# JuliaPhysics/BeamletOptics.jl

Hardware: AMD Instinct MI355X
Metric: ray-surface intersections/s (higher is better)
Workload: dtype f64

## Files before the change

### beamletoptics.jl_amd/csrc/bmo_engine.hip

```cpp
#include <hip/hip_runtime.h>
#include <hipcub/hipcub.hpp>

#include <algorithm>
#include <cmath>
#include <chrono>
#include <cstdio>
#include <cstdlib>
#include <cstring>
#include <ctime>
#include <unistd.h>
#include <memory>
#include <mutex>
#include <string>
#include <map>
#include <vector>

#include "bmo_lane.hpp"

using namespace bmo;

namespace {

thread_local std::string g_err;
struct Knobs {
// ... 1274 lines not shown
        c0.d[L::OPL * cap + j] = 0.0;
    }
    c0.i[I_NODE * cap + j] = perm ? perm[j] : (int32_t)j;
    c0.i[I_K * cap + j] = 0;
    c0.i[I_HOBJ * cap + j] = -1;
    c0.i[I_HSHAPE * cap + j] = -1;
    c0.i[I_FLAGS * cap + j] = (1 < r_max) ? 0 : F_DEAD;
    if (KIND == BMO_BEAM_GAUSSIAN) {
        nodes.aux[j * 4 + 0] = cont ? planes[27 * n + j] : 0.0;
        nodes.aux[j * 4 + 1] = planes[20 * n + j];
        nodes.aux[j * 4 + 2] = planes[21 * n + j];
        nodes.aux[j * 4 + 3] = planes[22 * n + j];
    }
    nodes.root[j] = (int32_t)j;
    nodes.parent[j] = -1;
    nodes.nseg[j] = 1;
    nodes.status[j] = 0;
    nodes.li[j] = lambda_idx[j];
    nodes.lambda[j] = planes[(KIND == BMO_BEAM_GAUSSIAN ? 18 : 6) * n + j];
    nodes.hit_det[j] = -1;
    nodes.key[j] = 0;
    if (nodes.tbits) nodes.tbits[j] = 1ull;
}
__global__ void bin_planes_kernel(const double* __restrict__ in, const int32_t* __restrict__ perm, int64_t n, int n_planes, double* __restrict__ out) {
    const int64_t s = (int64_t)blockIdx.x * blockDim.x + threadIdx.x;
    if (s >= n) return;
    const int64_t j = perm[s];
    for (int p = 0; p < n_planes; ++p) out[(int64_t)p * n + s] = in[(int64_t)p * n + j];
}

__global__ void old_obj_scatter_kernel(Chunk c, int32_t chunk_index, const int32_t* __restrict__ rec_start, int32_t* __restrict__ rec_obj,
                                       int64_t* __restrict__ rec_loc) {
    const int64_t j = (int64_t)blockIdx.x * blockDim.x + threadIdx.x;
    if (j >= c.count) return;
    const int32_t node = chunk_node(c, j);
    if (node < 0) return;
    const int32_t k = c.i[I_K * c.cap + j];
    rec_obj[(int64_t)rec_start[node] + k] = c.i[I_OBJ * c.cap + j];
    rec_loc[(int64_t)rec_start[node] + k] = ((int64_t)chunk_index << OLD_LOC_SHIFT) | j;
}
__global__ void old_first_child_kernel(const int32_t* __restrict__ parent, const unsigned long long* __restrict__ key, int64_t n, int32_t* __restrict__ first_child) {
    const int64_t c = (int64_t)blockIdx.x * blockDim.x + threadIdx.x;
    if (c >= n) return;
    const int32_t p = parent[c];
    if (p >= 0 && !(key[c] & 1ull)) first_child[p] = (int32_t)c;
}
constexpr int MAX_PATH_LEVELS = 26;
__global__ void pack_keys_kernel(const int32_t* __restrict__ root_of, const unsigned long long* __restrict__ key, int64_t n, int bits_depth, int bits_path,
                                 uint32_t* __restrict__ k32, unsigned long long* __restrict__ k64) {
    const int64_t i = (int64_t)blockIdx.x * blockDim.x + threadIdx.x;
    if (i >= n) return;
    const unsigned long long k = key[i];
    const unsigned long long root = (unsigned long long)root_of[i], depth = k >> 32, path = k & ((1ull << bits_path) - 1ull);
    const unsigned long long packed = (root << (bits_depth + bits_path)) | (depth << bits_path) | path;
    if (k32) k32[i] = (uint32_t)packed;
    else k64[i] = packed;
}
constexpr int MAX_HEAP_LEVELS = 5;
__device__ __forceinline__ unsigned heap_index(unsigned long long key) {
    const unsigned depth = (unsigned)(key >> 32);
    return (1u << depth) - 1u + (unsigned)(key & ((1ull << depth) - 1ull));
}
__global__ void tree_bits_kernel(const int32_t* __restrict__ root_of, const unsigned long long* __restrict__ key, int64_t n, unsigned long long* __restrict__ bits) {
    const int64_t i = (int64_t)blockIdx.x * blockDim.x + threadIdx.x;
    if (i >= n) return;
    atomicOr(&bits[root_of[i]], 1ull << heap_index(key[i]));
}
__global__ void tree_count_kernel(const unsigned long long* __restrict__ bits, int64_t n_roots, int32_t* __restrict__ cnt) {
    const int64_t r = (int64_t)blockIdx.x * blockDim.x + threadIdx.x;
    if (r < n_roots) cnt[r] = __popcll(bits[r]);
}
__global__ void tree_rank_kernel(const int32_t* __restrict__ root_of, const unsigned long long* __restrict__ key, int64_t n, const unsigned long long* __restrict__ bits,
                                 const int32_t* __restrict__ base, int32_t* __restrict__ order) {
    const int64_t i = (int64_t)blockIdx.x * blockDim.x + threadIdx.x;
    if (i >= n) return;
    const int32_t r = root_of[i];
    const unsigned h = heap_index(key[i]);
    order[base[r] + __popcll(bits[r] & ((1ull << h) - 1ull))] = (int32_t)i;
}
__global__ void node_depth_kernel(const unsigned long long* __restrict__ key, int64_t n, uint32_t* __restrict__ depth) {
    const int64_t i = (int64_t)blockIdx.x * blockDim.x + threadIdx.x;
    if (i < n) depth[i] = (uint32_t)(key[i] >> 32);
}
__global__ void level_starts_kernel(const uint32_t* __restrict__ sorted_depth, int64_t n, int64_t max_depth, int32_t* __restrict__ start) {
    const int64_t i = (int64_t)blockIdx.x * blockDim.x + threadIdx.x;
    if (i >= n) return;
    const int64_t d = sorted_depth[i], dprev = i ? (int64_t)sorted_depth[i - 1] : -1;
    for (int64_t x = dprev + 1; x <= d; ++x) start[x] = (int32_t)i;
    if (i == n - 1)
        for (int64_t x = d + 1; x <= max_depth + 1; ++x) start[x] = (int32_t)n;
}
__global__ void level_root_rank_kernel(const int32_t* __restrict__ ids, int32_t cnt, int32_t* __restrict__ rank) {
    const int i = blockIdx.x * blockDim.x + threadIdx.x;
    if (i < cnt) rank[ids[i]] = i;
}
__global__ void level_flag_kernel(const int32_t* __restrict__ ids, int32_t cnt, const int32_t* __restrict__ parent, const unsigned long long* __restrict__ key,
                                  const int32_t* __restrict__ rank, int32_t* __restrict__ flag) {
    const int i = blockIdx.x * blockDim.x + threadIdx.x;
    if (i >= cnt) return;
    const int32_t nd = ids[i];
    if (!(key[nd] & 1ull)) flag[rank[parent[nd]]] = 1;
}
__global__ void level_rank_kernel(const int32_t* __restrict__ ids, int32_t cnt, const int32_t* __restrict__ parent, const unsigned long long* __restrict__ key,
                                  const int32_t* __restrict__ scan, int32_t* __restrict__ rank) {
    const int i = blockIdx.x * blockDim.x + threadIdx.x;
    if (i >= cnt) return;
    const int32_t nd = ids[i];
    rank[nd] = 2 * scan[rank[parent[nd]]] + (int32_t)(key[nd] & 1ull);
}
__global__ void gather_u32_kernel(const int32_t* __restrict__ idx, const int32_t* __restrict__ src, int64_t n, uint32_t* __restrict__ dst) {
    const int64_t i = (int64_t)blockIdx.x * blockDim.x + threadIdx.x;
    if (i < n) dst[i] = (uint32_t)src[idx[i]];
}
__global__ void root_depth_key_kernel(const int32_t* __restrict__ idx, const int32_t* __restrict__ root_of, const unsigned long long* __restrict__ key, int64_t n,
                                      int bits_depth, unsigned long long* __restrict__ out) {
    const int64_t i = (int64_t)blockIdx.x * blockDim.x + threadIdx.x;
    if (i >= n) return;
    const int32_t nd = idx[i];
    out[i] = ((unsigned long long)root_of[nd] << bits_depth) | (key[nd] >> 32);
}
__global__ void iota_kernel(int32_t* a, int64_t n) {
    const int64_t j = (int64_t)blockIdx.x * blockDim.x + threadIdx.x;
    if (j < n) a[j] = (int32_t)j;
}
__global__ void sweep_key_kernel(Chunk c, const int32_t* __restrict__ root, const int32_t* __restrict__ root_cfg, int64_t m, uint32_t* __restrict__ key,
                                 int32_t* __restrict__ slot) {
    const int64_t j = (int64_t)blockIdx.x * blockDim.x + threadIdx.x;
    if (j >= m) return;
    key[j] = (uint32_t)root_cfg[root[c.i[I_NODE * c.cap + j]]];
    slot[j] = (int32_t)j;
}
__global__ void sweep_bounds_kernel(const uint32_t* __restrict__ key, int64_t m, int32_t* __restrict__ beg, int32_t* __restrict__ end) {
    const int64_t i = (int64_t)blockIdx.x * blockDim.x + threadIdx.x;
    if (i >= m) return;
    const uint32_t k = key[i];
    if (i == 0 || key[i - 1] != k) beg[k] = (int32_t)i;
    if (i == m - 1 || key[i + 1] != k) end[k] = (int32_t)(i + 1);
}
__global__ void sweep_pad_kernel(const int32_t* __restrict__ beg, const int32_t* __restrict__ end, int32_t n_configs, int32_t* __restrict__ padded) {
    const int32_t c = (int32_t)(blockIdx.x * blockDim.x + threadIdx.x);
    if (c >= n_configs) return;
    padded[c] = (end[c] - beg[c] + 63) & ~63;
}
__global__ void sweep_scatter_kernel(const uint32_t* __restrict__ key, const int32_t* __restrict__ slot, int64_t m, const int32_t* __restrict__ beg,
                                     const int32_t* __restrict__ pstart, int64_t lanes, int32_t* __restrict__ map, unsigned long long* __restrict__ overflow) {
    const int64_t i = (int64_t)blockIdx.x * blockDim.x + threadIdx.x;
    if (i >= m) return;
    const uint32_t k = key[i];
    const int64_t v = (int64_t)pstart[k] + (i - beg[k]);
    if (v < lanes) map[v] = slot[i];
    else atomicAdd(overflow, 1ull);
}

__global__ void hit_flags_kernel(const int32_t* order, const int32_t* hit_det, int64_t n, int32_t n_det, int32_t nsub, int32_t* flags) {
    const int64_t i = (int64_t)blockIdx.x * blockDim.x + threadIdx.x;
    if (i >= n) return;
    const int32_t d = hit_det[order[i]];
    for (int32_t q = 0; q < n_det; ++q) flags[(int64_t)q * n + i] = (q == d) ? nsub : 0;
}
__global__ void hit_offsets_kernel(const int32_t* __restrict__ offs, const int32_t* __restrict__ flags, int64_t n, int32_t n_det, int32_t* __restrict__ out) {
    const int d = (int)threadIdx.x;
    if (d < n_det) out[d] = offs[(int64_t)d * n];
    if (d == n_det) out[d] = offs[(int64_t)n_det * n - 1] + flags[(int64_t)n_det * n - 1];
}
__global__ void hit_gather_kernel(const int32_t* __restrict__ order, const int32_t* __restrict__ hit_det, const double* __restrict__ hit, int64_t n, int32_t nsub,
                                  const int32_t* __restrict__ offs, int64_t cap, double* __restrict__ out, int32_t* __restrict__ out_node,
                                  unsigned long long* __restrict__ overflow) {
    __shared__ int32_t s_nd[256], s_pos[256];
    const int64_t i0 = (int64_t)blockIdx.x * 256;
    {
        const int64_t i = i0 + threadIdx.x;
        int32_t nd = -1, pos = -1;
        if (i < n) {
            nd = order[i];
            const int32_t d = hit_det[nd];
            if (d >= 0) {
                pos = offs[(int64_t)d * n + i];
                if ((int64_t)pos + nsub > cap) {
                    atomicAdd(overflow, 1ull);
                    pos = -1;
                } else {
                    for (int q = 0; q < nsub; ++q) out_node[pos + q] = (int32_t)i;
                }
            }
        }
        s_nd[threadIdx.x] = nd;
        s_pos[threadIdx.x] = pos;
    }
    __syncthreads();
    const int width = 9 * nsub;
    const int de = 256 / width, dk = 256 % width;
    int e = (int)threadIdx.x / width, k = (int)threadIdx.x % width;
    for (int t = threadIdx.x; t < 256 * width; t += 256) {
        const int32_t pos = s_pos[e];
        if (pos >= 0) out[(int64_t)pos * 9 + k] = hit[(int64_t)s_nd[e] * width + k];
        e += de;
        k += dk;
        if (k >= width) {
            k -= width;
            e += 1;
        }
    }
}

__global__ void rank_kernel(const int32_t* __restrict__ order, int64_t n, int32_t* __restrict__ rank) {
    const int64_t i = (int64_t)blockIdx.x * blockDim.x + threadIdx.x;
    if (i < n) rank[order[i]] = (int32_t)i;
}
__global__ void canon_nodes_kernel(const int32_t* __restrict__ order, const int32_t* __restrict__ rank, int64_t n, int gaussian, const int32_t* __restrict__ root,
                                   const int32_t* __restrict__ parent, const int32_t* __restrict__ nseg, const int32_t* __restrict__ status,
                                   const unsigned long long* __restrict__ key, const double* __restrict__ lambda, const double* __restrict__ aux,
                                   int32_t* __restrict__ o_root, int32_t* __restrict__ o_parent, int32_t* __restrict__ o_first_child, int32_t* __restrict__ o_nseg,
                                   int32_t* __restrict__ o_status, double* __restrict__ o_aux) {
    const int64_t i = (int64_t)blockIdx.x * blockDim.x + threadIdx.x;
    if (i >= n) return;
    const int32_t nd = order[i];
    const int32_t p = parent[nd];
    o_root[i] = root[nd];
    o_parent[i] = p < 0 ? -1 : rank[p];
    o_nseg[i] = nseg[nd];
    o_status[i] = status[nd];
    if (gaussian) {
        o_aux[4 * i + 0] = aux[4 * (int64_t)nd + 1];
        o_aux[4 * i + 1] = aux[4 * (int64_t)nd + 2];
        o_aux[4 * i + 2] = aux[4 * (int64_t)nd + 3];
        o_aux[4 * i + 3] = lambda[nd];
    } else {
        o_aux[4 * i + 0] = lambda[nd];
        o_aux[4 * i + 1] = o_aux[4 * i + 2] = o_aux[4 * i + 3] = 0.0;
    }
    if (p >= 0 && !(key[nd] & 1ull)) o_first_child[rank[p]] = (int32_t)i;
}
__global__ void dst_base_kernel(const int32_t* __restrict__ order, const int32_t* __restrict__ first_rec, int64_t n, int32_t* __restrict__ dst_base) {
    const int64_t i = (int64_t)blockIdx.x * blockDim.x + threadIdx.x;
    if (i < n) dst_base[order[i]] = first_rec[i];
}
__global__ void last_records_kernel(Chunk c, int planes, const int32_t* __restrict__ rank, const int32_t* __restrict__ nseg, int64_t nn, double* __restrict__ rec,
                                    int32_t* __restrict__ obj, int32_t* __restrict__ shape) {
    const int64_t j = (int64_t)blockIdx.x * blockDim.x + threadIdx.x;
    if (j >= c.count) return;
    const int32_t nd = chunk_node(c, j);
    if (nd < 0) return;
    if (c.i[I_K * c.cap + j] != nseg[nd] - 1) return;
    const int64_t dst = rank[nd];
    for (int p = 0; p < planes; ++p) rec[(int64_t)p * nn + dst] = c.d[(int64_t)p * c.cap + j];
    obj[dst] = c.i[I_OBJ * c.cap + j];
    shape[dst] = c.i[I_SHAPE * c.cap + j];
}
__global__ void hit_columns_kernel(const double* __restrict__ src, int64_t n, int n_cols, double* __restrict__ dst) {
    const int64_t t = (int64_t)blockIdx.x * blockDim.x + threadIdx.x;
    if (t >= n * n_cols) return;
    const int64_t i = t / n_cols;
    dst[t] = src[i * 9 + (t - i * n_cols)];
}

__global__ void order_records_kernel(Chunk c, int planes, const int32_t* __restrict__ dst_base, int64_t nr, double* __restrict__ rec,
                                     int32_t* __restrict__ obj, int32_t* __restrict__ shape) {
    const int64_t j = (int64_t)blockIdx.x * blockDim.x + threadIdx.x;
    if (j >= c.count) return;
    const int32_t nd = chunk_node(c, j);
    if (nd < 0) return;
    const int64_t dst = (int64_t)dst_base[nd] + c.i[I_K * c.cap + j];
    for (int p = 0; p < planes; ++p) rec[(int64_t)p * nr + dst] = c.d[(int64_t)p * c.cap + j];
    obj[dst] = c.i[I_OBJ * c.cap + j];
    shape[dst] = c.i[I_SHAPE * c.cap + j];
}

struct PoolBlock {
    void* p;
    size_t bytes;
    int device;
};
std::mutex g_pool_mu;
std::vector<PoolBlock> g_pool;
size_t g_pool_bytes = 0;

void* pool_take(size_t bytes, int device, size_t& got) {
    std::lock_guard<std::mutex> lk(g_pool_mu);
    int best = -1;
    for (int i = 0; i < (int)g_pool.size(); ++i) {
        const PoolBlock& b = g_pool[i];
        if (b.device != device || b.bytes < bytes || b.bytes > bytes + bytes / 4 + 4096) continue;
        if (best < 0 || b.bytes < g_pool[best].bytes) best = i;
    }
    if (best < 0) return nullptr;
    void* p = g_pool[best].p;
    got = g_pool[best].bytes;
    g_pool_bytes -= got;
    g_pool.erase(g_pool.begin() + best);
    return p;
}
void pool_give(void* p, size_t bytes, int device) {
    std::lock_guard<std::mutex> lk(g_pool_mu);
    g_pool.push_back({p, bytes, device});
    g_pool_bytes += bytes;
}
void pool_release_all() {
    std::lock_guard<std::mutex> lk(g_pool_mu);
    int cur = 0;
    (void)hipGetDevice(&cur);
    for (auto& b : g_pool) {
        (void)hipSetDevice(b.device);
        (void)hipFree(b.p);
    }
    (void)hipSetDevice(cur);
    g_pool.clear();
    g_pool_bytes = 0;
}

struct PoolHold;
thread_local PoolHold* g_hold = nullptr;
void host_pool_give(void* p, size_t bytes);
struct PoolHold {
    hipStream_t stream;
    std::vector<PoolBlock> dev;
    std::vector<std::pair<void*, size_t>> host;
    PoolHold* prev;
    explicit PoolHold(hipStream_t s) : stream(s), prev(g_hold) { g_hold = this; }
    ~PoolHold() {
        g_hold = prev;
        (void)hipStreamSynchronize(stream);
        for (auto& b : dev) pool_give(b.p, b.bytes, b.device);
        for (auto& h : host) host_pool_give(h.first, h.second);
    }
    PoolHold(const PoolHold&) = delete;
    PoolHold& operator=(const PoolHold&) = delete;
    struct Now {
        PoolHold* saved;
        Now() : saved(g_hold) { g_hold = nullptr; }
        ~Now() { g_hold = saved; }
    };
};

struct DevBuf {
    void* p = nullptr;
    size_t bytes = 0;
// ... 1179 lines not shown
```

### beamletoptics.jl_amd/csrc/bmo_trace_host.inc.hpp

```cpp

struct DevCtx {
    hipStream_t stream = nullptr;
    hipEvent_t ev[4] = {nullptr, nullptr, nullptr, nullptr};
    Counters* pinned = nullptr;
    std::vector<hipEvent_t> step_ev;
    std::mutex busy;
};
int device_ctx(int device, DevCtx*& out) {
    static std::mutex ctx_mu;
    static std::vector<std::pair<int, std::unique_ptr<DevCtx>>> ctxs;
    std::lock_guard<std::mutex> lk(ctx_mu);
    for (auto& c : ctxs)
        if (c.first == device) {
            out = c.second.get();
            return BMO_OK;
        }
    auto nc = std::make_unique<DevCtx>();
    HIP_TRY(hipStreamCreateWithFlags(&nc->stream, hipStreamNonBlocking));
    for (int q = 0; q < 4; ++q) HIP_TRY(hipEventCreate(&nc->ev[q]));
    HIP_TRY(hipHostMalloc(reinterpret_cast<void**>(&nc->pinned), sizeof(Counters), hipHostMallocDefault));
    out = nc.get();
    ctxs.emplace_back(device, std::move(nc));
    return BMO_OK;
}
// ... 343 lines not shown
    const double span = (double)(t1 - t0);
    const int NB = 40;
    std::vector<double> busy(NB, 0.0);
    for (size_t w = 0; w < nw; ++w) {
        const double a = (double)(t[2 * w] - t0) / span * NB, b2 = (double)(t[2 * w + 1] - t0) / span * NB;
        for (int q = (int)a; q < NB && q <= (int)b2; ++q) busy[q] += std::min(b2, (double)q + 1) - std::max(a, (double)q);
    }
    fprintf(stderr, "[bmo] timeline step %d: %zu waves, span %.3f ms; mean waves at work per 1/%d of the span:\n ", steps, nw, span / 1e5, NB);
    for (int q = 0; q < NB; ++q) fprintf(stderr, " %.0f", busy[q]);
    fprintf(stderr, "\n");
    {
        std::vector<size_t> idx(nw);
        for (size_t w = 0; w < nw; ++w) idx[w] = w;
        const size_t top = std::min<size_t>(nw, 12);
        std::partial_sort(idx.begin(), idx.begin() + (long)top, idx.end(), [&](size_t a, size_t b2) { return t[2 * a + 1] > t[2 * b2 + 1]; });
        fprintf(stderr, "[bmo] timeline step %d: last waves to end (wave of the grid: start .. end in ms):", steps);
        for (size_t q = 0; q < top; ++q) fprintf(stderr, "  %zu: %.3f .. %.3f", idx[q], (double)(t[2 * idx[q]] - t0) / 1e5, (double)(t[2 * idx[q] + 1] - t0) / 1e5);
        fprintf(stderr, "\n");
        std::vector<double> dur(nw);
        for (size_t w = 0; w < nw; ++w) dur[w] = (double)(t[2 * w + 1] - t[2 * w]) / 1e5;
        std::vector<double> srt = dur;
        std::sort(srt.begin(), srt.end());
        fprintf(stderr, "[bmo] timeline step %d: wave durations ms p50 %.3f p90 %.3f p99 %.3f p99.9 %.3f max %.3f\n", steps, srt[nw / 2], srt[nw * 9 / 10], srt[nw * 99 / 100],
                srt[std::min(nw - 1, nw * 999 / 1000)], srt[nw - 1]);
    }
    return BMO_OK;
}
#endif

int launch_step(DevCtx& ctx, const StepKernels& kern, const LaunchPlan& plan, const StepParams& P, int step, Counters* d_ctr) {
    hipStream_t stream = ctx.stream;
    while ((int)ctx.step_ev.size() < 2 * (step + 1)) {
        hipEvent_t e;
        HIP_TRY(hipEventCreate(&e));
        ctx.step_ev.push_back(e);
    }
    HIP_TRY(hipEventRecord(ctx.step_ev[2 * step], stream));
    const char* const wide_env = getenv("BMO_WIDE_MIN_WAVES");
    const int64_t wide_min_waves = wide_env ? atoll(wide_env) : 4096;
    const bool wide = kern.plain_wide && plan.n_waves >= wide_min_waves;
    const StepKernel k = (plan.inwave_cap > 0 && kern.inw) ? (wide ? kern.inw_wide : kern.inw) : (wide ? kern.plain_wide : kern.plain);
    if (!k) return fail(BMO_ERR_INTERNAL, "no step kernel selected for this beam kind / scene level");
    DBG("step %d kernel build: %s, %s", step, wide ? "4 waves per SIMD" : "default waves per SIMD", (plan.inwave_cap > 0 && kern.inw) ? "in-loop splitters" : "splits end the loop");
    hipLaunchKernelGGL(k, dim3(plan.n_blocks), dim3(BMO_BLOCK), STEP_LDS_BYTES, stream, P);
    HIP_TRY(hipEventRecord(ctx.step_ev[2 * step + 1], stream));
    HIP_TRY(hipMemcpyAsync(ctx.pinned, d_ctr, sizeof(Counters), hipMemcpyDeviceToHost, stream));
    HIP_TRY(hipStreamSynchronize(stream));
    HIP_TRY(hipGetLastError());
    return BMO_OK;
}

inline int bits_for(unsigned long long v) {
    int b = 0;
    while (b < 64 && (v >> b)) ++b;
    return b;
}

int order_by_heap_index(bmo_trace_result* R, int64_t n, int64_t n_nodes, const DevBuf& tbits, hipStream_t stream, Temps& temps) {
    DevBuf *bits = temps.take((size_t)n * 8), *cnt = temps.take((size_t)n * 4), *base = temps.take((size_t)n * 4);
    if (!bits || !cnt || !base) return BMO_ERR_OOM;
    const unsigned nb = (unsigned)((n_nodes + 255) / 256), rb = (unsigned)((n + 255) / 256);
    const unsigned long long* b = (const unsigned long long*)(tbits.p ? tbits.p : bits->p);
    if (!tbits.p) {
        HIP_TRY(hipMemsetAsync(bits->p, 0, (size_t)n * 8, stream));
        hipLaunchKernelGGL(tree_bits_kernel, dim3(nb), dim3(256), 0, stream, (const int32_t*)R->n_root.p, (const unsigned long long*)R->n_key.p, n_nodes,
                           (unsigned long long*)bits->p);
    }
    hipLaunchKernelGGL(tree_count_kernel, dim3(rb), dim3(256), 0, stream, b, n, (int32_t*)cnt->p);
    CUB_TRY(temps, hipcub::DeviceScan::ExclusiveSum(cub_tmp, cub_bytes, (const int32_t*)cnt->p, (int32_t*)base->p, (int)n, stream));
    hipLaunchKernelGGL(tree_rank_kernel, dim3(nb), dim3(256), 0, stream, (const int32_t*)R->n_root.p, (const unsigned long long*)R->n_key.p, n_nodes, b,
                       (const int32_t*)base->p, (int32_t*)R->order.p);
    return BMO_OK;
}

int order_by_packed_keys(bmo_trace_result* R, int64_t n_nodes, int bits_root, int bits_depth, int bits_path, hipStream_t stream, Temps& temps) {
    const int bits = bits_root + bits_depth + bits_path;
    const bool narrow = bits <= 32;
    DevBuf *k_in = temps.take((size_t)n_nodes * (narrow ? 4 : 8)), *k_out = temps.take((size_t)n_nodes * (narrow ? 4 : 8)), *v_out = temps.take((size_t)n_nodes * 4);
    if (!k_in || !k_out || !v_out) return BMO_ERR_OOM;
    hipLaunchKernelGGL(pack_keys_kernel, dim3((unsigned)((n_nodes + 255) / 256)), dim3(256), 0, stream, (const int32_t*)R->n_root.p, (const unsigned long long*)R->n_key.p,
                       n_nodes, bits_depth, bits_path, narrow ? (uint32_t*)k_in->p : nullptr, narrow ? nullptr : (unsigned long long*)k_in->p);
    if (narrow)
        CUB_TRY(temps, hipcub::DeviceRadixSort::SortPairs(cub_tmp, cub_bytes, (const uint32_t*)k_in->p, (uint32_t*)k_out->p, (const int32_t*)R->order.p, (int32_t*)v_out->p,
                                                          (int)n_nodes, 0, bits, stream));
    else
        CUB_TRY(temps, hipcub::DeviceRadixSort::SortPairs(cub_tmp, cub_bytes, (const unsigned long long*)k_in->p, (unsigned long long*)k_out->p, (const int32_t*)R->order.p,
                                                          (int32_t*)v_out->p, (int)n_nodes, 0, bits, stream));
    std::swap(R->order.p, v_out->p);
    std::swap(R->order.bytes, v_out->bytes);
    return BMO_OK;
}

int order_level_by_level(bmo_trace_result* R, int64_t n_nodes, int64_t md, int bits_root, int bits_depth, hipStream_t stream) {
    int rc;
    const unsigned nb = (unsigned)((n_nodes + 255) / 256);
    const int32_t* parent = (const int32_t*)R->n_parent.p;
    const unsigned long long* key = (const unsigned long long*)R->n_key.p;
    DevBuf depth, depth_sorted, by_depth, starts, rank, flag, scan, k64, k64_out, ids2, keys_in, keys_out, vals_out;
    Temps tmp;
    if ((rc = depth.alloc((size_t)n_nodes * 4)) || (rc = depth_sorted.alloc((size_t)n_nodes * 4)) || (rc = by_depth.alloc((size_t)n_nodes * 4)) ||
        (rc = starts.alloc((size_t)(md + 2) * 4)) || (rc = rank.alloc((size_t)n_nodes * 4)) || (rc = flag.alloc((size_t)n_nodes * 4)) ||
        (rc = scan.alloc((size_t)n_nodes * 4)) || (rc = k64.alloc((size_t)n_nodes * 8)) || (rc = k64_out.alloc((size_t)n_nodes * 8)) ||
        (rc = ids2.alloc((size_t)n_nodes * 4)) || (rc = vals_out.alloc((size_t)n_nodes * 4)) || (rc = keys_in.alloc((size_t)n_nodes * 4)) ||
        (rc = keys_out.alloc((size_t)n_nodes * 4)))
        return rc;
    hipLaunchKernelGGL(node_depth_kernel, dim3(nb), dim3(256), 0, stream, key, n_nodes, (uint32_t*)depth.p);
    CUB_TRY(tmp, hipcub::DeviceRadixSort::SortPairs(cub_tmp, cub_bytes, (const uint32_t*)depth.p, (uint32_t*)depth_sorted.p, (const int32_t*)R->order.p, (int32_t*)by_depth.p,
                                                    (int)n_nodes, 0, bits_depth, stream));
    hipLaunchKernelGGL(level_starts_kernel, dim3(nb), dim3(256), 0, stream, (const uint32_t*)depth_sorted.p, n_nodes, md, (int32_t*)starts.p);
    std::vector<int32_t> h_start((size_t)md + 2);
    HIP_TRY(hipMemcpyAsync(h_start.data(), starts.p, (size_t)(md + 2) * 4, hipMemcpyDeviceToHost, stream));
    HIP_TRY(hipStreamSynchronize(stream));
    const int32_t* ids = (const int32_t*)by_depth.p;
    hipLaunchKernelGGL(level_root_rank_kernel, dim3((unsigned)((h_start[1] + 255) / 256)), dim3(256), 0, stream, ids, h_start[1], (int32_t*)rank.p);
    int32_t max_level = h_start[1];
    for (int64_t d = 1; d <= md; ++d) {
        const int32_t cnt_prev = h_start[d] - h_start[d - 1], cnt = h_start[d + 1] - h_start[d];
        if (cnt <= 0 || cnt_prev <= 0) continue;
        max_level = std::max(max_level, cnt);
        const unsigned lb = (unsigned)((cnt + 255) / 256);
        HIP_TRY(hipMemsetAsync(flag.p, 0, (size_t)cnt_prev * 4, stream));
        hipLaunchKernelGGL(level_flag_kernel, dim3(lb), dim3(256), 0, stream, ids + h_start[d], cnt, parent, key, (const int32_t*)rank.p, (int32_t*)flag.p);
        CUB_TRY(tmp, hipcub::DeviceScan::ExclusiveSum(cub_tmp, cub_bytes, (const int32_t*)flag.p, (int32_t*)scan.p, (int)cnt_prev, stream));
        hipLaunchKernelGGL(level_rank_kernel, dim3(lb), dim3(256), 0, stream, ids + h_start[d], cnt, parent, key, (const int32_t*)scan.p, (int32_t*)rank.p);
    }
    hipLaunchKernelGGL(gather_u32_kernel, dim3(nb), dim3(256), 0, stream, (const int32_t*)R->order.p, (const int32_t*)rank.p, n_nodes, (uint32_t*)keys_in.p);
    CUB_TRY(tmp, hipcub::DeviceRadixSort::SortPairs(cub_tmp, cub_bytes, (const uint32_t*)keys_in.p, (uint32_t*)keys_out.p, (const int32_t*)R->order.p, (int32_t*)ids2.p,
                                                    (int)n_nodes, 0, bits_for((unsigned long long)max_level), stream));
    hipLaunchKernelGGL(root_depth_key_kernel, dim3(nb), dim3(256), 0, stream, (const int32_t*)ids2.p, (const int32_t*)R->n_root.p, key, n_nodes, bits_depth,
                       (unsigned long long*)k64.p);
    CUB_TRY(tmp, hipcub::DeviceRadixSort::SortPairs(cub_tmp, cub_bytes, (const unsigned long long*)k64.p, (unsigned long long*)k64_out.p, (const int32_t*)ids2.p,
                                                    (int32_t*)vals_out.p, (int)n_nodes, 0, bits_root + bits_depth, stream));
    HIP_TRY(hipGetLastError());
    HIP_TRY(hipStreamSynchronize(stream));
    std::swap(R->order.p, vals_out.p);
    std::swap(R->order.bytes, vals_out.bytes);
    return BMO_OK;
}

int order_nodes(bmo_trace_result* R, int64_t n, int64_t n_nodes, unsigned long long max_depth, const DevBuf& tbits, hipStream_t stream, Temps& temps) {
    int rc;
    if ((rc = R->order.alloc((size_t)std::max<int64_t>(n_nodes, 1) * 4))) return rc;
    const bool force_deep = std::getenv("BMO_FORCE_DEEP_ORDER") != nullptr;
    if (n_nodes > n && max_depth <= (unsigned long long)MAX_HEAP_LEVELS && !std::getenv("BMO_FORCE_SORT_ORDER") && !force_deep)
        return order_by_heap_index(R, n, n_nodes, tbits, stream, temps);
    if (n_nodes > 0) hipLaunchKernelGGL(iota_kernel, dim3((unsigned)((n_nodes + 255) / 256)), dim3(256), 0, stream, (int32_t*)R->order.p, n_nodes);
    if (n_nodes <= n) return BMO_OK;
    const int bits_depth = bits_for(max_depth), bits_root = bits_for((unsigned long long)std::max<int64_t>(n - 1, 0));
    if (max_depth <= (unsigned long long)MAX_PATH_LEVELS && !force_deep)
        return order_by_packed_keys(R, n_nodes, bits_root, bits_depth, (int)max_depth , stream, temps);
    return order_level_by_level(R, n_nodes, (int64_t)max_depth, bits_root, bits_depth, stream);
}

int gather_detector_hits(bmo_trace_result* R, int nsub, int64_t n, int64_t n_nodes, Counters* d_ctr, int32_t* h_off, hipStream_t stream, Temps& temps) {
    int rc;
    const int nd = R->n_detectors;
    const int64_t tot = (int64_t)nd * n_nodes;
    if (tot >= ((int64_t)1 << 31)) return fail(BMO_ERR_UNSUPPORTED, "detectors x beams exceeds 2^31: split the batch");
    if (nd + 1 > 1024) return fail(BMO_ERR_UNSUPPORTED, "more than 1023 detectors");
    DevBuf *flags = temps.take((size_t)tot * 4), *offs = temps.take((size_t)tot * 4), *d_off = temps.take((size_t)(nd + 1) * 4);
    if (!flags || !offs || !d_off) return BMO_ERR_OOM;
    const unsigned nb = (unsigned)((n_nodes + 255) / 256);
    hipLaunchKernelGGL(hit_flags_kernel, dim3(nb), dim3(256), 0, stream, (const int32_t*)R->order.p, (const int32_t*)R->n_hitdet.p, n_nodes, nd, nsub,
                       (int32_t*)flags->p);
    CUB_TRY(temps, hipcub::DeviceScan::ExclusiveSum(cub_tmp, cub_bytes, (const int32_t*)flags->p, (int32_t*)offs->p, (int)tot, stream));
    hipLaunchKernelGGL(hit_offsets_kernel, dim3(1), dim3(1024), 0, stream, (const int32_t*)offs->p, (const int32_t*)flags->p, n_nodes, nd, (int32_t*)d_off->p);
    HIP_TRY(hipMemcpyAsync(h_off, d_off->p, (size_t)(nd + 1) * 4, hipMemcpyDeviceToHost, stream));
    const int64_t bound = (n_nodes + n) / 2 * nsub + nsub;
    if ((rc = R->det_data.alloc((size_t)std::max<int64_t>(bound, 1) * 72)) || (rc = R->det_node.alloc((size_t)std::max<int64_t>(bound, 1) * 4))) return rc;
    hipLaunchKernelGGL(hit_gather_kernel, dim3(nb), dim3(256), 0, stream, (const int32_t*)R->order.p, (const int32_t*)R->n_hitdet.p, (const double*)R->n_hit.p,
                       n_nodes, nsub, (const int32_t*)offs->p, bound, (double*)R->det_data.p, (int32_t*)R->det_node.p, &d_ctr->overflow);
    return BMO_OK;
}

void note_detector_kinds(const bmo_scene* scene, bmo_trace_result* R) {
    R->det_kind.assign((size_t)R->n_detectors, -1);
    const bmo_object* obj = reinterpret_cast<const bmo_object*>(scene->blob.data() + scene->hdr.off_objects);
    for (int i = 0; i < scene->hdr.n_objects; ++i) {
        const int k = obj[i].kind, d = obj[i].detector;
        if ((k == BMO_OBJ_SPOTDETECTOR || k == BMO_OBJ_PSFDETECTOR || k == BMO_OBJ_PHOTODETECTOR) && d >= 0 && d < R->n_detectors)
            R->det_kind[(size_t)d] = (R->det_kind[(size_t)d] == -1 || R->det_kind[(size_t)d] == k) ? k : -2;
    }
}

OldSolution old_solution_of(const bmo_trace_result* prev) {
    OldSolution o{};
    o.nseg = (const int32_t*)prev->n_nseg.p;
    o.status = (const int32_t*)prev->n_status.p;
    o.first_child = (const int32_t*)prev->rt_first_child.p;
    o.rec_start = (const int32_t*)prev->rt_rec_start.p;
    o.rec_obj = (const int32_t*)prev->rt_rec_obj.p;
    o.aux = (const double*)prev->n_aux.p;
    o.rec_loc = (const int64_t*)prev->rt_rec_loc.p;
    o.chunks = (const OldChunk*)prev->rt_chunks.p;
    return o;
}

int alloc_launch_chunks(const KindInfo& K, ChunkArena& arena, bmo_trace_result* R, LaunchPlan& plan, bool has_split, LaunchChunks& C, ChunkArena::Mark* marks) {
    int rc;
    const int64_t m = C.cur.count;
    const bool sweep = plan.sweep_lanes > 0;
    if ((rc = arena.alloc((has_split ? 2 * m : m) + plan.inwave_cap + (plan.keep_kids ? m : 0), C.nxt))) return rc;
    C.wl = nullptr;
    if (arena.keep_log && plan.n_fuse > 1) {
        auto b = std::make_unique<DevBuf>();
        if ((rc = b->alloc(sweep ? (size_t)m : (size_t)plan.n_blocks * (BMO_BLOCK / 64)))) return rc;
        C.wl = static_cast<uint8_t*>(b->p);
        R->wave_last.push_back(std::move(b));
    }
    marks[0] = arena.mark();
    for (int q = 0; q < (K.gauss ? plan.n_fuse : plan.n_fuse - 1); ++q) {
        if (!arena.keep_log && q > (K.gauss ? 1 : 0)) {
            C.inner[q] = C.inner[K.gauss ? (q & 1) : 0];
            continue;
        }
        if ((rc = arena.alloc(m, C.inner[q]))) {
            if (rc != BMO_ERR_OOM || q == 0) return rc;
            plan.n_fuse = K.gauss ? q : q + 1;
            break;
        }
        C.inner[q].count = m;
        C.inner[q].wl = C.wl;
        C.inner[q].level = q + 1;
        C.inner[q].wl_shift = sweep ? 0 : plan.lane_shift;
        marks[q + 1] = arena.mark();
    }
    C.n_inner = K.gauss ? plan.n_fuse : plan.n_fuse - 1;
    return BMO_OK;
}

int run_trace(const KindInfo& K, bmo_scene* scene, bmo_device_batch* batch, const bmo_trace_opts* opts, bmo_trace_result* R, bmo_trace_result* prev) {
    const int device = batch->device;
    if (prev) {
        if (prev->device != device) return fail(BMO_ERR_INVALID, "retrace: the previous solution lives on another device");
        if (prev->kind != K.kind || prev->n_roots != batch->n)
            return fail(BMO_ERR_INVALID, "retrace: batch does not match the previous solution (root count / beam kind)");
    }
    HIP_TRY(hipSetDevice(device));
    int rc = BMO_OK;
    const char* dblob = scene->device_blob(device, rc);
    if (rc) return rc;
    const int64_t n = batch->n;
    const bool has_split = scene->hdr.has_splitter != 0;
    R->device = device;
    R->kind = K.kind;
    R->n_roots = n;
    R->n_detectors = scene->hdr.n_detectors;
    note_detector_kinds(scene, R);
    R->nd = K.nd;
    R->abi_planes = K.abi_planes;

    auto wall0 = std::chrono::steady_clock::now();
    auto lap = [&](const char* what) {
        if (!dbg_on()) return;
        auto t = std::chrono::steady_clock::now();
        DBG("phase %-10s %.3f ms", what, std::chrono::duration<double, std::milli>(t - wall0).count());
        wall0 = t;
    };
    DevCtx* ctxp = nullptr;
    if ((rc = device_ctx(device, ctxp))) return rc;
    DevCtx& ctx = *ctxp;
    std::lock_guard<std::mutex> one_trace_per_device(ctx.busy);
    hipStream_t stream = ctx.stream;
    hipEvent_t ev_t0 = ctx.ev[2], ev_t1 = ctx.ev[3];
    HIP_TRY(hipEventRecord(ev_t0, stream));
    PoolHold hold(stream);

    NodeTable nodes{R, K.nsub, prev != nullptr};
    if ((rc = nodes.alloc(has_split ? (n <= ((int64_t)1 << 22) ? 7 * n + 64 : 3 * n + 64) : n))) return rc;
    DevBuf tbits_buf;

    const bool keep_log = opts->record_segments != 0;
    R->has_log = keep_log;
    const size_t rec_bytes = (size_t)K.nd * 8 + (size_t)NI * 4;
    ChunkArena arena{R->arena, (size_t)K.nd * 8, rec_bytes, std::max<size_t>((size_t)n * rec_bytes * 6, (size_t)1 << 20), keep_log};

    DevBuf ctr_buf, shard_buf;
    if ((rc = ctr_buf.alloc(sizeof(Counters))) || (rc = shard_buf.alloc(64 * 128))) return rc;
    HIP_TRY(hipMemsetAsync(shard_buf.p, 0, 64 * 128, stream));
    Counters* d_ctr = static_cast<Counters*>(ctr_buf.p);
    Counters& h_ctr = *ctx.pinned;
    h_ctr = Counters{{0, 0}, (unsigned long long)n, 0, 0, {0, 0}};
    HIP_TRY(hipMemcpyAsync(d_ctr, &h_ctr, sizeof h_ctr, hipMemcpyHostToDevice, stream));

    LaunchChunks C;
    if ((rc = arena.alloc(n, C.cur))) return rc;
    C.cur.count = n;
    OldSolution old_tab{};
    if (prev) {
        if ((rc = build_retrace_tables(prev, stream))) return rc;
        old_tab = old_solution_of(prev);
    }
    if (has_split && n > 0 && (rc = tbits_buf.alloc((size_t)n * 8))) return rc;
    if (n > 0) {
        hipLaunchKernelGGL(K.init_roots, dim3((unsigned)((n + 255) / 256)), dim3(256), 0, stream, (const double*)batch->planes.p,
                           (const double*)(batch->perm.p ? batch->binned.p : batch->planes.p), (const int32_t*)batch->li.p, (const int32_t*)batch->perm.p, n, C.cur,
                           nodes.arrays(tbits_buf), prev ? 0x7fffffff : opts->r_max, (int32_t)batch->n_planes);
        if (prev) hipLaunchKernelGGL(iota_kernel, dim3((unsigned)((n + 255) / 256)), dim3(256), 0, stream, (int32_t*)R->n_old.p, n);
    }
    lap("setup");
    DBG("roots initialised n=%lld blob=%u use_lds=%d", (long long)n, (uint32_t)scene->blob.size(), 0);
    if (dbg_on()) {
        HIP_TRY(hipStreamSynchronize(stream));
        HIP_TRY(hipGetLastError());
        DBG("init kernel done");
    }
    const bool sweep = R->n_configs > 0;
    StepKernels kern;
    const int ext = scene->hdr.pad[0] ? 3 : (scene->hdr.has_asphere ? 2 : (scene->hdr.has_meniscus ? 1 : 0));
    if ((rc = K.select(ext, prev != nullptr, sweep, kern))) return rc;

    int64_t n_nodes = n;
    int steps = 0;
    int fuse_max = K.gauss ? MAX_FUSE - 1 : MAX_FUSE;
    if (const char* e = getenv(K.gauss ? "BMO_FUSE_GAUSS" : "BMO_FUSE")) fuse_max = std::max(1, std::min(fuse_max, atoi(e)));
    LaunchBufs bufs;
    while (C.cur.count > 0) {
        const int64_t m = C.cur.count;
        LaunchPlan plan = plan_launch(m, fuse_max, keep_log, rec_bytes, has_split, kern.inw || K.gauss, R->n_configs);
        if (plan.sweep_lanes >= ((int64_t)1 << 31)) return fail(BMO_ERR_UNSUPPORTED, "sweep launch of more than 2^31 lanes: fewer roots per call");
        ChunkArena::Mark marks[MAX_FUSE];
        if ((rc = alloc_launch_chunks(K, arena, R, plan, has_split, C, marks))) return rc;
        if (has_split && (rc = nodes.grow(n_nodes + 2 * m + 2 * plan.inwave_cap, stream))) return rc;
        if ((rc = bufs.fit(K, plan, m, rec_bytes))) return rc;
        StepParams P;
        fill_step_params(P, K, scene, dblob, opts, C, plan, bufs, nodes.arrays(tbits_buf), old_tab, d_ctr, shard_buf.p, steps, n_nodes);
        if (knobs().lpt && !sweep && steps == 0 && plan.lane_shift == 6 && plan.n_blocks >= 64 && (rc = tile_order_feedback(P, batch, prev, plan.n_blocks, stream))) return rc;
#if defined(BMO_DEV_TIMELINE)
        DevBuf tl_buf;
        if (getenv("BMO_TIMELINE") && !sweep) {
            if ((rc = tl_buf.alloc((size_t)plan.n_waves * 16 + 64))) return rc;
            HIP_TRY(hipMemsetAsync(tl_buf.p, 0, tl_buf.bytes, stream));
            P.tl = (unsigned long long*)tl_buf.p;
        }
#endif
        DevBuf sw_map;
        if (sweep) {
            if ((rc = build_sweep_lane_map(R, C.cur, plan.sweep_lanes, d_ctr, stream, sw_map))) return rc;
            P.sweep = SweepLanes{(const int32_t*)sw_map.p, (const int32_t*)R->d_root_cfg.p, scene->stride};
        }
        DBG("step %d launching m=%lld, %d records per wave", steps, (long long)m, 1 << plan.lane_shift);
        if ((rc = launch_step(ctx, kern, plan, P, steps, d_ctr))) return rc;
#if defined(BMO_DEV_TIMELINE)
        if (P.tl && (rc = print_timeline(P.tl, (size_t)plan.n_waves, steps))) return rc;
#endif
        const unsigned long long produced = h_ctr.next_count[steps & 1];
        DBG("step %d done next=%llu nodes=%llu deepest in-place level %llu of %d", steps, produced, h_ctr.node_count, h_ctr.max_level[steps & 1], plan.n_fuse);
        steps += 1;
        if (h_ctr.overflow) return fail(BMO_ERR_INTERNAL, "queue overflow (internal capacity bound violated)");
        if (h_ctr.sweep_mixed) return fail(BMO_ERR_INTERNAL, "sweep: a wave held records of more than one configuration (lane map violated)");
        if (keep_log) {
            const int used = (int)std::min<unsigned long long>(h_ctr.max_level[(steps - 1) & 1], (unsigned long long)(plan.n_fuse - 1));
            R->chunks.push_back(C.cur);
            for (int q = 0; q < used; ++q) R->chunks.push_back(C.inner[q]);
            if (used < C.n_inner) arena.rewind(marks[used]);
        } else {
            arena.drop(C.cur);
            if (K.gauss || plan.n_fuse > 1) arena.drop(C.inner[0]);
            if (K.gauss && plan.n_fuse > 1) arena.drop(C.inner[1]);
        }
        C.nxt.count = (int64_t)produced;
        n_nodes = (int64_t)h_ctr.node_count;
        if (opts->max_beams > 0 && n_nodes > (int64_t)opts->max_beams)
            return fail(BMO_ERR_LIMIT, "beam tree exceeds bmo_trace_opts.max_beams (" + std::to_string(n_nodes) + " beams after " + std::to_string(steps) +
                                           " launches): a splitter facing a mirror?");
        C.cur = C.nxt;
    }
    double kernel_ms = 0;
    for (int q = 0; q < steps; ++q) {
        float ms = 0;
        HIP_TRY(hipEventElapsedTime(&ms, ctx.step_ev[2 * q], ctx.step_ev[2 * q + 1]));
        kernel_ms += ms;
        DBG("step %d kernel %.3f ms", q, ms);
        if (q + 1 < steps && getenv("BMO_GAPS")) {
            float gap = 0;
            (void)hipEventElapsedTime(&gap, ctx.step_ev[2 * q + 1], ctx.step_ev[2 * q + 2]);
            fprintf(stderr, "[bmo] step %d kernel %.3f ms, gap to the next launch %.3f ms\n", q, ms, gap);
        }
    }
    lap("steps");
    R->n_nodes = n_nodes;
    R->n_steps = steps;
    R->kernel_ms = kernel_ms;
    if (batch->cost_valid && batch->tile_n > 0 && batch->tile_cost.p && !R->tile_cost.alloc((size_t)batch->tile_n * 4)) {
        if (hipMemcpyAsync(R->tile_cost.p, batch->tile_cost.p, (size_t)batch->tile_n * 4, hipMemcpyDeviceToDevice, stream) == hipSuccess) R->tile_n = batch->tile_n;
    }
    Temps temps;
    static_assert(sizeof(unsigned long long) == 8, "");
    HostBuf h_tail;
    if ((rc = h_tail.alloc((1024 + 1 + 1025) * 8))) return rc;
    unsigned long long* const h_sh = static_cast<unsigned long long*>(h_tail.p);
    long long* const h_sum = reinterpret_cast<long long*>(h_sh + 1024);
    int32_t* const h_off = reinterpret_cast<int32_t*>(h_sh + 1025);
    *h_sum = 0;
    HIP_TRY(hipMemcpyAsync(h_sh, shard_buf.p, 64 * 128, hipMemcpyDeviceToHost, stream));
    if (n_nodes > 0) {
        DevBuf* d_sum = temps.take(8);
        if (!d_sum) return BMO_ERR_OOM;
        CUB_TRY(temps, hipcub::DeviceReduce::Sum(cub_tmp, cub_bytes, (const int32_t*)R->n_nseg.p, (long long*)d_sum->p, (int)n_nodes, stream));
        HIP_TRY(hipMemcpyAsync(h_sum, d_sum->p, 8, hipMemcpyDeviceToHost, stream));
    }
    if ((rc = order_nodes(R, n, n_nodes, h_ctr.max_depth, tbits_buf, stream, temps))) return rc;
    lap("order");
    const int nd = R->n_detectors;
    R->det_count.assign(nd, 0);
    R->det_offset.assign(nd, 0);
    const bool with_hits = nd > 0 && n_nodes > 0;
    if (with_hits && (rc = gather_detector_hits(R, K.nsub, n, n_nodes, d_ctr, h_off, stream, temps))) return rc;
    HIP_TRY(hipMemcpyAsync(&h_ctr, d_ctr, sizeof h_ctr, hipMemcpyDeviceToHost, stream));
    HIP_TRY(hipEventRecord(ev_t1, stream));
    HIP_TRY(hipStreamSynchronize(stream));
    HIP_TRY(hipGetLastError());
    lap("hits");
    if (h_ctr.overflow) return fail(BMO_ERR_INTERNAL, "hit table overflow (internal capacity bound violated)");
    {
        unsigned long long tot = 0;
        for (int q = 0; q < 64; ++q) tot += h_sh[(size_t)q * 16];
        R->calls = tot;
        R->n_records = (int64_t)*h_sum;
    }
    if (with_hits)
        for (int d = 0; d < nd; ++d) {
            R->det_offset[d] = h_off[d];
            R->det_count[d] = h_off[d + 1] - h_off[d];
        }
    float tms = 0;
    HIP_TRY(hipEventElapsedTime(&tms, ev_t0, ev_t1));
    R->total_ms = tms;
    return BMO_OK;
}

int trace_by_kind(bmo_scene* scene, bmo_device_batch* batch, const bmo_trace_opts* opts, bmo_trace_result* R, bmo_trace_result* prev) {
    if (batch->kind == BMO_BEAM_RAY) return run_trace(kind_info<BMO_BEAM_RAY>(), scene, batch, opts, R, prev);
    if (batch->kind == BMO_BEAM_POLARIZED) return run_trace(kind_info<BMO_BEAM_POLARIZED>(), scene, batch, opts, R, prev);
    if (batch->kind == BMO_BEAM_GAUSSIAN) return run_trace(kind_info<BMO_BEAM_GAUSSIAN>(), scene, batch, opts, R, prev);
    return fail(BMO_ERR_UNSUPPORTED, "beam kind not built yet");
}
```

Baseline: 45.30 billion.

## Replace per-detector flag scan with block histogram ranks and batch tail readbacks

Detector-hit compaction no longer writes an n_det × n_nodes flag array and scans it. Each block now counts hits per detector with wavefront ballots into shared memory, and only an n_det × n_blocks table is scanned. The gather kernel recomputes in-block ranks to place each hit, and block 0 writes the detector offsets. The segment-count reduction is fused into the count kernel through an atomic. Counters, shards, segment sum and offsets now share one device tail buffer read back with a single copy. This cuts scan traffic and the number of small D2H copies and launches, at the cost of duplicated rank work and more complex kernels.

```diff
diff --git a/beamletoptics.jl_amd/csrc/bmo_engine.hip b/beamletoptics.jl_amd/csrc/bmo_engine.hip
--- a/beamletoptics.jl_amd/csrc/bmo_engine.hip
+++ b/beamletoptics.jl_amd/csrc/bmo_engine.hip
@@ -1450,36 +1450,72 @@
     else atomicAdd(overflow, 1ull);
 }
 
-__global__ void hit_flags_kernel(const int32_t* order, const int32_t* hit_det, int64_t n, int32_t n_det, int32_t nsub, int32_t* flags) {
-    const int64_t i = (int64_t)blockIdx.x * blockDim.x + threadIdx.x;
-    if (i >= n) return;
-    const int32_t d = hit_det[order[i]];
-    for (int32_t q = 0; q < n_det; ++q) flags[(int64_t)q * n + i] = (q == d) ? nsub : 0;
-}
-__global__ void hit_offsets_kernel(const int32_t* __restrict__ offs, const int32_t* __restrict__ flags, int64_t n, int32_t n_det, int32_t* __restrict__ out) {
-    const int d = (int)threadIdx.x;
-    if (d < n_det) out[d] = offs[(int64_t)d * n];
-    if (d == n_det) out[d] = offs[(int64_t)n_det * n - 1] + flags[(int64_t)n_det * n - 1];
-}
-__global__ void hit_gather_kernel(const int32_t* __restrict__ order, const int32_t* __restrict__ hit_det, const double* __restrict__ hit, int64_t n, int32_t nsub,
-                                  const int32_t* __restrict__ offs, int64_t cap, double* __restrict__ out, int32_t* __restrict__ out_node,
-                                  unsigned long long* __restrict__ overflow) {
+__device__ __forceinline__ int32_t block_hit_rank(int32_t d, int32_t n_det, int32_t* hist) {
+    const int w = (int)threadIdx.x >> 6, lane = (int)threadIdx.x & 63;
+    for (int q = (int)threadIdx.x; q < 4 * n_det; q += 256) hist[q] = 0;
+    __syncthreads();
+    int32_t r = 0;
+    unsigned long long todo = __ballot(d >= 0);
+    while (todo) {
+        const int lead = __ffsll(todo) - 1;
+        const int32_t dq = __shfl(d, lead);
+        const unsigned long long m = __ballot(d == dq);
+        if (d == dq) r = __popcll(m & ((1ull << lane) - 1));
+        if (lane == lead) hist[w * n_det + dq] = __popcll(m);
+        todo &= ~m;
+    }
+    __syncthreads();
+    if (d >= 0)
+        for (int v = 0; v < w; ++v) r += hist[v * n_det + d];
+    return r;
+}
+__global__ __launch_bounds__(256) void hit_count_kernel(const int32_t* __restrict__ order, const int32_t* __restrict__ hit_det, const int32_t* __restrict__ nseg,
+                                                        int64_t n, int32_t n_det, int32_t nsub, int32_t n_blocks, int32_t* __restrict__ table,
+                                                        unsigned long long* __restrict__ seg_sum) {
+    extern __shared__ int32_t s_hist[];
+    __shared__ long long s_seg[4];
+    const int64_t i = (int64_t)blockIdx.x * 256 + threadIdx.x;
+    int32_t d = -1;
+    long long seg = 0;
+    if (i < n) {
+        d = hit_det[order[i]];
+        if (d >= n_det) d = -1;
+        seg = nseg[i];
+    }
+    (void)block_hit_rank(d, n_det, s_hist);
+    for (int q = (int)threadIdx.x; q < n_det; q += 256)
+        table[(int64_t)q * n_blocks + blockIdx.x] = nsub * (s_hist[q] + s_hist[n_det + q] + s_hist[2 * n_det + q] + s_hist[3 * n_det + q]);
+    for (int s = 32; s > 0; s >>= 1) seg += __shfl_down(seg, s);
+    if ((threadIdx.x & 63) == 0) s_seg[threadIdx.x >> 6] = seg;
+    __syncthreads();
+    if (threadIdx.x == 0) atomicAdd(seg_sum, (unsigned long long)(s_seg[0] + s_seg[1] + s_seg[2] + s_seg[3]));
+}
+__global__ __launch_bounds__(256) void hit_gather_kernel(const int32_t* __restrict__ order, const int32_t* __restrict__ hit_det, const double* __restrict__ hit, int64_t n,
+                                                         int32_t n_det, int32_t nsub, int32_t n_blocks, const int32_t* __restrict__ base,
+                                                         const int32_t* __restrict__ table, int64_t cap, double* __restrict__ out, int32_t* __restrict__ out_node,
+                                                         int32_t* __restrict__ out_offsets, unsigned long long* __restrict__ overflow) {
+    extern __shared__ int32_t s_hist[];
     __shared__ int32_t s_nd[256], s_pos[256];
     const int64_t i0 = (int64_t)blockIdx.x * 256;
+    if (blockIdx.x == 0)
+        for (int q = (int)threadIdx.x; q <= n_det; q += 256)
+            out_offsets[q] = q < n_det ? base[(int64_t)q * n_blocks] : base[(int64_t)n_det * n_blocks - 1] + table[(int64_t)n_det * n_blocks - 1];
     {
         const int64_t i = i0 + threadIdx.x;
-        int32_t nd = -1, pos = -1;
+        int32_t nd = -1, pos = -1, d = -1;
         if (i < n) {
             nd = order[i];
-            const int32_t d = hit_det[nd];
-            if (d >= 0) {
-                pos = offs[(int64_t)d * n + i];
-                if ((int64_t)pos + nsub > cap) {
-                    atomicAdd(overflow, 1ull);
-                    pos = -1;
-                } else {
-                    for (int q = 0; q < nsub; ++q) out_node[pos + q] = (int32_t)i;
-                }
+            d = hit_det[nd];
+            if (d >= n_det) d = -1;
+        }
+        const int32_t r = block_hit_rank(d, n_det, s_hist);
+        if (d >= 0) {
+            pos = base[(int64_t)d * n_blocks + blockIdx.x] + r * nsub;
+            if ((int64_t)pos + nsub > cap) {
+                atomicAdd(overflow, 1ull);
+                pos = -1;
+            } else {
+                for (int q = 0; q < nsub; ++q) out_node[pos + q] = (int32_t)i;
             }
         }
         s_nd[threadIdx.x] = nd;
diff --git a/beamletoptics.jl_amd/csrc/bmo_trace_host.inc.hpp b/beamletoptics.jl_amd/csrc/bmo_trace_host.inc.hpp
--- a/beamletoptics.jl_amd/csrc/bmo_trace_host.inc.hpp
+++ b/beamletoptics.jl_amd/csrc/bmo_trace_host.inc.hpp
@@ -519,24 +519,25 @@
     return order_level_by_level(R, n_nodes, (int64_t)max_depth, bits_root, bits_depth, stream);
 }
 
-int gather_detector_hits(bmo_trace_result* R, int nsub, int64_t n, int64_t n_nodes, Counters* d_ctr, int32_t* h_off, hipStream_t stream, Temps& temps) {
+int gather_detector_hits(bmo_trace_result* R, int nsub, int64_t n, int64_t n_nodes, Counters* d_ctr, int32_t* d_off, unsigned long long* d_seg, hipStream_t stream,
+                         Temps& temps) {
     int rc;
     const int nd = R->n_detectors;
-    const int64_t tot = (int64_t)nd * n_nodes;
-    if (tot >= ((int64_t)1 << 31)) return fail(BMO_ERR_UNSUPPORTED, "detectors x beams exceeds 2^31: split the batch");
+    if ((int64_t)nd * n_nodes >= ((int64_t)1 << 31)) return fail(BMO_ERR_UNSUPPORTED, "detectors x beams exceeds 2^31: split the batch");
     if (nd + 1 > 1024) return fail(BMO_ERR_UNSUPPORTED, "more than 1023 detectors");
-    DevBuf *flags = temps.take((size_t)tot * 4), *offs = temps.take((size_t)tot * 4), *d_off = temps.take((size_t)(nd + 1) * 4);
-    if (!flags || !offs || !d_off) return BMO_ERR_OOM;
     const unsigned nb = (unsigned)((n_nodes + 255) / 256);
-    hipLaunchKernelGGL(hit_flags_kernel, dim3(nb), dim3(256), 0, stream, (const int32_t*)R->order.p, (const int32_t*)R->n_hitdet.p, n_nodes, nd, nsub,
-                       (int32_t*)flags->p);
-    CUB_TRY(temps, hipcub::DeviceScan::ExclusiveSum(cub_tmp, cub_bytes, (const int32_t*)flags->p, (int32_t*)offs->p, (int)tot, stream));
-    hipLaunchKernelGGL(hit_offsets_kernel, dim3(1), dim3(1024), 0, stream, (const int32_t*)offs->p, (const int32_t*)flags->p, n_nodes, nd, (int32_t*)d_off->p);
-    HIP_TRY(hipMemcpyAsync(h_off, d_off->p, (size_t)(nd + 1) * 4, hipMemcpyDeviceToHost, stream));
+    const int64_t tot = (int64_t)nd * nb;
+    DevBuf *table = temps.take((size_t)tot * 4), *base = temps.take((size_t)tot * 4);
+    if (!table || !base) return BMO_ERR_OOM;
+    const size_t lds = (size_t)4 * nd * 4;
+    hipLaunchKernelGGL(hit_count_kernel, dim3(nb), dim3(256), lds, stream, (const int32_t*)R->order.p, (const int32_t*)R->n_hitdet.p, (const int32_t*)R->n_nseg.p,
+                       n_nodes, nd, nsub, (int32_t)nb, (int32_t*)table->p, d_seg);
+    CUB_TRY(temps, hipcub::DeviceScan::ExclusiveSum(cub_tmp, cub_bytes, (const int32_t*)table->p, (int32_t*)base->p, (int)tot, stream));
     const int64_t bound = (n_nodes + n) / 2 * nsub + nsub;
     if ((rc = R->det_data.alloc((size_t)std::max<int64_t>(bound, 1) * 72)) || (rc = R->det_node.alloc((size_t)std::max<int64_t>(bound, 1) * 4))) return rc;
-    hipLaunchKernelGGL(hit_gather_kernel, dim3(nb), dim3(256), 0, stream, (const int32_t*)R->order.p, (const int32_t*)R->n_hitdet.p, (const double*)R->n_hit.p,
-                       n_nodes, nsub, (const int32_t*)offs->p, bound, (double*)R->det_data.p, (int32_t*)R->det_node.p, &d_ctr->overflow);
+    hipLaunchKernelGGL(hit_gather_kernel, dim3(nb), dim3(256), lds, stream, (const int32_t*)R->order.p, (const int32_t*)R->n_hitdet.p, (const double*)R->n_hit.p,
+                       n_nodes, nd, nsub, (int32_t)nb, (const int32_t*)base->p, (const int32_t*)table->p, bound, (double*)R->det_data.p, (int32_t*)R->det_node.p,
+                       d_off, &d_ctr->overflow);
     return BMO_OK;
 }
 
@@ -595,6 +596,9 @@
     C.n_inner = K.gauss ? plan.n_fuse : plan.n_fuse - 1;
     return BMO_OK;
 }
+
+constexpr size_t TAIL_CTR = 0, TAIL_SHARDS = 128, TAIL_SEG = TAIL_SHARDS + 64 * 128, TAIL_OFF = TAIL_SEG + 8, TAIL_BYTES = (TAIL_OFF + 1025 * 4 + 127) / 128 * 128;
+static_assert(sizeof(Counters) <= TAIL_SHARDS, "Counters has the first 128 bytes of the tail block");
 
 int run_trace(const KindInfo& K, bmo_scene* scene, bmo_device_batch* batch, const bmo_trace_opts* opts, bmo_trace_result* R, bmo_trace_result* prev) {
     const int device = batch->device;
@@ -642,10 +646,12 @@
     const size_t rec_bytes = (size_t)K.nd * 8 + (size_t)NI * 4;
     ChunkArena arena{R->arena, (size_t)K.nd * 8, rec_bytes, std::max<size_t>((size_t)n * rec_bytes * 6, (size_t)1 << 20), keep_log};
 
-    DevBuf ctr_buf, shard_buf;
-    if ((rc = ctr_buf.alloc(sizeof(Counters))) || (rc = shard_buf.alloc(64 * 128))) return rc;
-    HIP_TRY(hipMemsetAsync(shard_buf.p, 0, 64 * 128, stream));
-    Counters* d_ctr = static_cast<Counters*>(ctr_buf.p);
+    DevBuf tail_buf;
+    if ((rc = tail_buf.alloc(TAIL_BYTES))) return rc;
+    HIP_TRY(hipMemsetAsync(tail_buf.p, 0, TAIL_BYTES, stream));
+    char* const d_tail = static_cast<char*>(tail_buf.p);
+    Counters* d_ctr = reinterpret_cast<Counters*>(d_tail + TAIL_CTR);
+    void* const d_shards = d_tail + TAIL_SHARDS;
     Counters& h_ctr = *ctx.pinned;
     h_ctr = Counters{{0, 0}, (unsigned long long)n, 0, 0, {0, 0}};
     HIP_TRY(hipMemcpyAsync(d_ctr, &h_ctr, sizeof h_ctr, hipMemcpyHostToDevice, stream));
@@ -691,7 +697,7 @@
         if (has_split && (rc = nodes.grow(n_nodes + 2 * m + 2 * plan.inwave_cap, stream))) return rc;
         if ((rc = bufs.fit(K, plan, m, rec_bytes))) return rc;
         StepParams P;
-        fill_step_params(P, K, scene, dblob, opts, C, plan, bufs, nodes.arrays(tbits_buf), old_tab, d_ctr, shard_buf.p, steps, n_nodes);
+        fill_step_params(P, K, scene, dblob, opts, C, plan, bufs, nodes.arrays(tbits_buf), old_tab, d_ctr, d_shards, steps, n_nodes);
         if (knobs().lpt && !sweep && steps == 0 && plan.lane_shift == 6 && plan.n_blocks >= 64 && (rc = tile_order_feedback(P, batch, prev, plan.n_blocks, stream))) return rc;
 #if defined(BMO_DEV_TIMELINE)
         DevBuf tl_buf;
@@ -753,38 +759,34 @@
         if (hipMemcpyAsync(R->tile_cost.p, batch->tile_cost.p, (size_t)batch->tile_n * 4, hipMemcpyDeviceToDevice, stream) == hipSuccess) R->tile_n = batch->tile_n;
     }
     Temps temps;
-    static_assert(sizeof(unsigned long long) == 8, "");
     HostBuf h_tail;
-    if ((rc = h_tail.alloc((1024 + 1 + 1025) * 8))) return rc;
-    unsigned long long* const h_sh = static_cast<unsigned long long*>(h_tail.p);
-    long long* const h_sum = reinterpret_cast<long long*>(h_sh + 1024);
-    int32_t* const h_off = reinterpret_cast<int32_t*>(h_sh + 1025);
-    *h_sum = 0;
-    HIP_TRY(hipMemcpyAsync(h_sh, shard_buf.p, 64 * 128, hipMemcpyDeviceToHost, stream));
-    if (n_nodes > 0) {
-        DevBuf* d_sum = temps.take(8);
-        if (!d_sum) return BMO_ERR_OOM;
-        CUB_TRY(temps, hipcub::DeviceReduce::Sum(cub_tmp, cub_bytes, (const int32_t*)R->n_nseg.p, (long long*)d_sum->p, (int)n_nodes, stream));
-        HIP_TRY(hipMemcpyAsync(h_sum, d_sum->p, 8, hipMemcpyDeviceToHost, stream));
-    }
+    if ((rc = h_tail.alloc(TAIL_BYTES))) return rc;
+    const char* const h_img = static_cast<const char*>(h_tail.p);
+    const unsigned long long* const h_sh = reinterpret_cast<const unsigned long long*>(h_img + TAIL_SHARDS);
+    const int32_t* const h_off = reinterpret_cast<const int32_t*>(h_img + TAIL_OFF);
+    unsigned long long* const d_seg = reinterpret_cast<unsigned long long*>(d_tail + TAIL_SEG);
+    const int nd = R->n_detectors;
+    const bool with_hits = nd > 0 && n_nodes > 0;
+    if (!with_hits && n_nodes > 0)
+        CUB_TRY(temps, hipcub::DeviceReduce::Sum(cub_tmp, cub_bytes, (const int32_t*)R->n_nseg.p, (long long*)d_seg, (int)n_nodes, stream));
     if ((rc = order_nodes(R, n, n_nodes, h_ctr.max_depth, tbits_buf, stream, temps))) return rc;
     lap("order");
-    const int nd = R->n_detectors;
     R->det_count.assign(nd, 0);
     R->det_offset.assign(nd, 0);
-    const bool with_hits = nd > 0 && n_nodes > 0;
-    if (with_hits && (rc = gather_detector_hits(R, K.nsub, n, n_nodes, d_ctr, h_off, stream, temps))) return rc;
-    HIP_TRY(hipMemcpyAsync(&h_ctr, d_ctr, sizeof h_ctr, hipMemcpyDeviceToHost, stream));
+    if (with_hits && (rc = gather_detector_hits(R, K.nsub, n, n_nodes, d_ctr, reinterpret_cast<int32_t*>(d_tail + TAIL_OFF), d_seg, stream, temps))) return rc;
+    HIP_TRY(hipMemcpyAsync(h_tail.p, d_tail, TAIL_BYTES, hipMemcpyDeviceToHost, stream));
     HIP_TRY(hipEventRecord(ev_t1, stream));
     HIP_TRY(hipStreamSynchronize(stream));
     HIP_TRY(hipGetLastError());
     lap("hits");
+    std::memcpy(&h_ctr, h_img + TAIL_CTR, sizeof h_ctr);
     if (h_ctr.overflow) return fail(BMO_ERR_INTERNAL, "hit table overflow (internal capacity bound violated)");
     {
-        unsigned long long tot = 0;
+        unsigned long long tot = 0, seg = 0;
         for (int q = 0; q < 64; ++q) tot += h_sh[(size_t)q * 16];
+        std::memcpy(&seg, h_img + TAIL_SEG, 8);
         R->calls = tot;
-        R->n_records = (int64_t)*h_sum;
+        R->n_records = (int64_t)seg;
     }
     if (with_hits)
         for (int d = 0; d < nd; ++d) {
```

Result: slower. 43.58 billion (-3.8%).
